# adr-arroyo/PointCloudComparator

Measured on AMD Instinct MI355X. Metric: nn_queries_per_sec, higher is better.
Workload: dtype f32; 1 GPU; C3: 10M x 10M XYZRGB (32-B stride), k=1 NN; step = index build over 10000000 references + 10000000 queries on each GPU (10000000 over 1 GPU); backend=none, engine=grid, references=10000000, queries_per_gpu=10000000, queries_total=10000000, point_stride_bytes=32

## Files before the change

pointcloudcomparator_amd/csrc/cellsort_mp.hip:

```cpp
#include "pcc_internal.hpp"
#include "grid_device.hpp"
#include "lane_ops.hpp"

namespace pcc {

constexpr int MP_T = 256;
constexpr unsigned int MP_F2 = 2048;
constexpr unsigned int MP_B2 = 128;
constexpr unsigned int MP_MAX_B1 = 256;
constexpr unsigned int MP_MAX_G = 512;
constexpr unsigned int MP_SLICE2 = 8192;
constexpr unsigned int MP_STAGE_BYTES = 32768;
constexpr unsigned int MP_WIN = 8;
#ifndef PCC_MP_STAGE_PTS
#define PCC_MP_STAGE_PTS 3072
#endif
#ifndef PCC_MP_STAGE_ORD
#define PCC_MP_STAGE_ORD 6144
#endif
constexpr unsigned int MP_FINE_STAGE_PTS = PCC_MP_STAGE_PTS, MP_FINE_STAGE_ORD = PCC_MP_STAGE_ORD;

struct MpPlan {
    unsigned int F1, F2, B1, G1, slice1;
};
static MpPlan mp_plan(unsigned int ncells_cap, unsigned int n) {
    MpPlan p;
    p.F2 = MP_F2;
    while ((unsigned long long)p.F2 * MP_B2 * MP_MAX_B1 < (unsigned long long)ncells_cap + 1) p.F2 *= 2;
    p.F1 = p.F2 * MP_B2;
    p.B1 = (ncells_cap + p.F1) / p.F1;
    p.G1 = (n + 16383) / 16384;
    if (p.G1 > MP_MAX_G) p.G1 = MP_MAX_G;
    if (p.G1 < 1) p.G1 = 1;
    p.slice1 = (n + p.G1 - 1) / p.G1;
    return p;
}

__device__ __forceinline__ unsigned int mp_cell(const float4& v, const GridParams& g, bool voxel) {
    return voxel ? voxel_id(v, g) : cell_id(v, g);
}
__device__ __forceinline__ unsigned int mp_cell(const uint2& v, const GridParams&, bool) { return v.x; }
__device__ __forceinline__ unsigned int mp_position(const float4& v) { return (unsigned int)__float_as_int(v.w); }
__device__ __forceinline__ unsigned int mp_position(const uint2& v) { return v.y; }
template <class E> __device__ __forceinline__ E mp_make(const float4& v, unsigned int cell);
template <> __device__ __forceinline__ float4 mp_make<float4>(const float4& v, unsigned int) { return v; }
template <> __device__ __forceinline__ uint2 mp_make<uint2>(const float4& v, unsigned int cell) {
    return make_uint2(cell, (unsigned int)__float_as_int(v.w));
}

__global__ void __launch_bounds__(MP_T)
k_mp_hist1(const float4* __restrict__ pts, unsigned int n, const GridDev* __restrict__ gd, unsigned int F1, unsigned int B1,
           unsigned int slice, unsigned int* __restrict__ H, unsigned int* __restrict__ zero, unsigned int n_zero) {
    for (unsigned int z = blockIdx.x * MP_T + threadIdx.x; z < n_zero; z += gridDim.x * MP_T) zero[z] = 0u;
    __shared__ unsigned int cnt[MP_MAX_B1];
    const GridParams g = gd->g;
    const bool voxel = gd->voxel != 0;
    for (unsigned int b = threadIdx.x; b < B1; b += MP_T) cnt[b] = 0;
    __syncthreads();
    const unsigned int beg = blockIdx.x * slice, end = min(n, beg + slice);
    for (unsigned int i0 = beg + threadIdx.x; i0 < end; i0 += 4 * MP_T) {
        float4 v[4];
#pragma unroll
        for (int u = 0; u < 4; ++u)
            if (i0 + u * MP_T < end) v[u] = pts[i0 + u * MP_T];
#pragma unroll
        for (int u = 0; u < 4; ++u)
            if (i0 + u * MP_T < end && __float_as_int(v[u].w) >= 0) atomicAdd(&cnt[mp_cell(v[u], g, voxel) / F1], 1u);
    }
    __syncthreads();
    for (unsigned int b = threadIdx.x; b < B1; b += MP_T) H[(size_t)b * gridDim.x + blockIdx.x] = cnt[b];
    if (blockIdx.x == 0 && threadIdx.x == 0) H[(size_t)B1 * gridDim.x] = 0;
}

template <class E>
__global__ void __launch_bounds__(MP_T)
k_mp_scatter1(const float4* __restrict__ pts, unsigned int n, const GridDev* __restrict__ gd, unsigned int F1, unsigned int B1,
              unsigned int slice, const unsigned int* __restrict__ H, E* __restrict__ out) {
    __shared__ unsigned int cur[MP_MAX_B1];
    const GridParams g = gd->g;
    const bool voxel = gd->voxel != 0;
    for (unsigned int b = threadIdx.x; b < B1; b += MP_T) cur[b] = H[(size_t)b * gridDim.x + blockIdx.x];
    __syncthreads();
    const unsigned int beg = blockIdx.x * slice, end = min(n, beg + slice);
    for (unsigned int i0 = beg + threadIdx.x; i0 < end; i0 += 4 * MP_T) {
        float4 v[4];
#pragma unroll
        for (int u = 0; u < 4; ++u)
            if (i0 + u * MP_T < end) v[u] = pts[i0 + u * MP_T];
#pragma unroll
        for (int u = 0; u < 4; ++u)
            if (i0 + u * MP_T < end && __float_as_int(v[u].w) >= 0) {
                const unsigned int c = mp_cell(v[u], g, voxel);
                out[atomicAdd(&cur[c / F1], 1u)] = mp_make<E>(v[u], c);
            }
    }
}

__global__ void __launch_bounds__(MP_T)
k_mp_hist1_cells(const unsigned int* __restrict__ cells, unsigned int n, unsigned int F1, unsigned int B1, unsigned int slice,
                 unsigned int* __restrict__ H, unsigned int* __restrict__ zero, unsigned int n_zero) {
    for (unsigned int z = blockIdx.x * MP_T + threadIdx.x; z < n_zero; z += gridDim.x * MP_T) zero[z] = 0u;
    __shared__ unsigned int cnt[MP_MAX_B1];
    for (unsigned int b = threadIdx.x; b < B1; b += MP_T) cnt[b] = 0;
    __syncthreads();
    const unsigned int beg = blockIdx.x * slice, end = min(n, beg + slice);
    for (unsigned int i0 = beg + threadIdx.x; i0 < end; i0 += 8 * MP_T) {
        unsigned int c[8];
#pragma unroll
        for (int u = 0; u < 8; ++u) c[u] = i0 + u * MP_T < end ? cells[i0 + u * MP_T] : 0xffffffffu;
#pragma unroll
        for (int u = 0; u < 8; ++u)
            if (c[u] != 0xffffffffu) atomicAdd(&cnt[c[u] / F1], 1u);
    }
    __syncthreads();
    for (unsigned int b = threadIdx.x; b < B1; b += MP_T) H[(size_t)b * gridDim.x + blockIdx.x] = cnt[b];
    if (blockIdx.x == 0 && threadIdx.x == 0) H[(size_t)B1 * gridDim.x] = 0;
}
__global__ void __launch_bounds__(MP_T)
k_mp_scatter1_cells(const unsigned int* __restrict__ cells, unsigned int n, unsigned int F1, unsigned int B1, unsigned int slice,
                    const unsigned int* __restrict__ H, uint2* __restrict__ out) {
    __shared__ unsigned int cur[MP_MAX_B1];
    for (unsigned int b = threadIdx.x; b < B1; b += MP_T) cur[b] = H[(size_t)b * gridDim.x + blockIdx.x];
    __syncthreads();
    const unsigned int beg = blockIdx.x * slice, end = min(n, beg + slice);
    for (unsigned int i0 = beg + threadIdx.x; i0 < end; i0 += 8 * MP_T) {
        unsigned int c[8];
#pragma unroll
        for (int u = 0; u < 8; ++u) c[u] = i0 + u * MP_T < end ? cells[i0 + u * MP_T] : 0xffffffffu;
#pragma unroll
        for (int u = 0; u < 8; ++u)
            if (c[u] != 0xffffffffu) out[atomicAdd(&cur[c[u] / F1], 1u)] = make_uint2(c[u], i0 + u * MP_T);
    }
}

constexpr unsigned int MP_TILE1 = 2048;
template <class E>
__global__ void __launch_bounds__(MP_T)
k_mp_scatter1_staged(const float4* __restrict__ pts, unsigned int n, const GridDev* __restrict__ gd, unsigned int F1, unsigned int B1,
                     unsigned int slice, const unsigned int* __restrict__ H, E* __restrict__ out) {
    constexpr int PER = MP_TILE1 / MP_T;
    __shared__ unsigned int cur[MP_MAX_B1], tcnt[MP_MAX_B1], tstart[MP_MAX_B1];
    __shared__ unsigned short sb[MP_TILE1];
    __shared__ __attribute__((aligned(16))) unsigned char stage_raw[MP_TILE1 * sizeof(E)];
    E* stage = reinterpret_cast<E*>(stage_raw);
    const GridParams g = gd->g;
    const bool voxel = gd->voxel != 0;
    for (unsigned int b = threadIdx.x; b < B1; b += MP_T) cur[b] = H[(size_t)b * gridDim.x + blockIdx.x];
    const unsigned int beg = blockIdx.x * slice, end = min(n, beg + slice);
    for (unsigned int t0 = beg; t0 < end; t0 += MP_TILE1) {
        for (unsigned int b = threadIdx.x; b < MP_MAX_B1; b += MP_T) tcnt[b] = 0;
        __syncthreads();
        float4 v[PER];
        unsigned int bk[PER], rk[PER];
#pragma unroll
        for (int u = 0; u < PER; ++u) {
            const unsigned int i = t0 + threadIdx.x + u * MP_T;
            v[u] = make_float4(0.f, 0.f, 0.f, __int_as_float(-1));
            if (i < end) v[u] = pts[i];
        }
#pragma unroll
        for (int u = 0; u < PER; ++u) {
            bk[u] = 0xffffffffu;
            rk[u] = 0;
            if (__float_as_int(v[u].w) >= 0) {
                bk[u] = mp_cell(v[u], g, voxel);
                rk[u] = atomicAdd(&tcnt[bk[u] / F1], 1u);
            }
        }
        __syncthreads();
        if (threadIdx.x < 64) {
            unsigned int c[4], sum = 0;
#pragma unroll
            for (int j = 0; j < 4; ++j) { c[j] = tcnt[4 * threadIdx.x + j]; sum += c[j]; }
            unsigned int ex = wave_incl_scan_add(sum) - sum;
#pragma unroll
            for (int j = 0; j < 4; ++j) { tstart[4 * threadIdx.x + j] = ex; ex += c[j]; }
        }
        __syncthreads();
#pragma unroll
        for (int u = 0; u < PER; ++u)
            if (bk[u] != 0xffffffffu) {
                const unsigned int b = bk[u] / F1, slot = tstart[b] + rk[u];
                stage[slot] = mp_make<E>(v[u], bk[u]);
                sb[slot] = (unsigned short)b;
            }
        __syncthreads();
        const unsigned int tile_n = tstart[MP_MAX_B1 - 1] + tcnt[MP_MAX_B1 - 1];
        for (unsigned int j = threadIdx.x; j < tile_n; j += MP_T) {
            const unsigned int b = sb[j];
            out[cur[b] + (j - tstart[b])] = stage[j];
        }
        __syncthreads();
        for (unsigned int b = threadIdx.x; b < MP_MAX_B1; b += MP_T) cur[b] += tcnt[b];
    }
}

__device__ __forceinline__ unsigned int mp_pair(unsigned int c, unsigned int F1, unsigned int F2) {
    return (c / F1) * MP_B2 + (c % F1) / F2;
}

template <bool PLACE, class E>
__global__ void __launch_bounds__(MP_T)
k_mp_level2(const E* __restrict__ in, const unsigned int* __restrict__ n_valid_ptr, const GridDev* __restrict__ gd,
            unsigned int F1, unsigned int F2, unsigned int* __restrict__ C, E* __restrict__ out) {
    constexpr unsigned int SLICE = PLACE ? MP_STAGE_BYTES / sizeof(E) : MP_SLICE2;
    __shared__ unsigned int cnt[MP_WIN * MP_B2];
    __shared__ __attribute__((aligned(16))) unsigned char stage_raw[PLACE ? MP_STAGE_BYTES : 16];
    E* stage = reinterpret_cast<E*>(stage_raw);
    const GridParams g = gd->g;
    const bool voxel = gd->voxel != 0;
    const unsigned int n = *n_valid_ptr;
    const unsigned int beg = blockIdx.x * SLICE, end = min(n, beg + SLICE);
    if (beg >= end) return;
    const unsigned int w0 = (mp_cell(in[beg], g, voxel) / F1) * MP_B2;
    for (unsigned int k = threadIdx.x; k < MP_WIN * MP_B2; k += MP_T) cnt[k] = 0;
    __syncthreads();
    for (unsigned int i0 = beg + threadIdx.x; i0 < end; i0 += 4 * MP_T) {
        E v[4];
#pragma unroll
        for (int u = 0; u < 4; ++u)
            if (i0 + u * MP_T < end) v[u] = in[i0 + u * MP_T];
#pragma unroll
        for (int u = 0; u < 4; ++u) {
            if (i0 + u * MP_T >= end) break;
            if (PLACE) stage[i0 + u * MP_T - beg] = v[u];
            const unsigned int pr = mp_pair(mp_cell(v[u], g, voxel), F1, F2);
            if (pr - w0 < MP_WIN * MP_B2) atomicAdd(&cnt[pr - w0], 1u);
            else if (!PLACE) atomicAdd(&C[pr], 1u);
            else out[atomicAdd(&C[pr], 1u)] = v[u];
        }
    }
    __syncthreads();
    for (unsigned int k = threadIdx.x; k < MP_WIN * MP_B2; k += MP_T) {
        const unsigned int c = cnt[k];
        if (c) {
            if (!PLACE) atomicAdd(&C[w0 + k], c);
            else cnt[k] = atomicAdd(&C[w0 + k], c);
        }
    }
    if (!PLACE) return;
    __syncthreads();
    for (unsigned int j = threadIdx.x; j < end - beg; j += MP_T) {
        const E v = stage[j];
        const unsigned int pr = mp_pair(mp_cell(v, g, voxel), F1, F2);
        if (pr - w0 < MP_WIN * MP_B2) out[atomicAdd(&cnt[pr - w0], 1u)] = v;
    }
}

__device__ __forceinline__ void mp_store_point(float4* out, unsigned int pos, const float4& v) { if (out) out[pos] = v; }
__device__ __forceinline__ void mp_store_point(float4*, unsigned int, const uint2&) {}

template <bool REFS, class E>
__global__ void __launch_bounds__(MP_T)
k_mp_fine(const E* __restrict__ in, const unsigned int* __restrict__ ends , const GridDev* __restrict__ gd,
          unsigned int F2, float4* __restrict__ out_pts, unsigned int* __restrict__ out_order,
          unsigned int* __restrict__ cell_start) {
    extern __shared__ __attribute__((aligned(16))) unsigned int lds[];
    unsigned int* cnt = lds;
    unsigned int* wsum = lds + F2;
    const GridParams g = gd->g;
    const bool voxel = gd->voxel != 0;
    const unsigned int ncells = (unsigned int)g.ncells;
    const unsigned int b = blockIdx.x;
    const unsigned int cell0 = b * F2;
    if (cell0 > ncells) return;
    const unsigned int beg = b ? ends[b - 1] : 0u, end = ends[b];
    if (!REFS && beg == end) return;
    for (unsigned int f = threadIdx.x; f < F2; f += MP_T) cnt[f] = 0;
    __syncthreads();
    for (unsigned int j0 = beg + threadIdx.x; j0 < end; j0 += 4 * MP_T) {
        E v[4];
#pragma unroll
        for (int u = 0; u < 4; ++u)
            if (j0 + u * MP_T < end) v[u] = in[j0 + u * MP_T];
#pragma unroll
        for (int u = 0; u < 4; ++u)
            if (j0 + u * MP_T < end) atomicAdd(&cnt[mp_cell(v[u], g, voxel) - cell0], 1u);
    }
    __syncthreads();
    const unsigned int per = (F2 + MP_T - 1) / MP_T;
    const unsigned int f0 = threadIdx.x * per, f1 = min(F2, f0 + per);
    unsigned int s = 0;
    for (unsigned int f = f0; f < f1; ++f) s += cnt[f];
    const unsigned int lane = threadIdx.x & 63, wave = threadIdx.x >> 6;
    const unsigned int inc = wave_incl_scan_add(s);
    if (lane == 63) wsum[wave] = inc;
    __syncthreads();
    unsigned int run = beg + inc - s;
    for (unsigned int w = 0; w < wave; ++w) run += wsum[w];
    for (unsigned int f = f0; f < f1; ++f) {
        const unsigned int c = cnt[f];
        cnt[f] = run;
        if (REFS && cell0 + f <= ncells) cell_start[cell0 + f] = run;
        run += c;
    }
    __syncthreads();
    const unsigned int stage_cap = out_pts ? MP_FINE_STAGE_PTS : MP_FINE_STAGE_ORD;
    const bool staged = end - beg <= stage_cap;
    float4* st_pts = reinterpret_cast<float4*>(lds + ((F2 + 4 + 3) & ~3u));
    unsigned int* st_ord = reinterpret_cast<unsigned int*>(st_pts + (out_pts ? MP_FINE_STAGE_PTS : 0));
    for (unsigned int j0 = beg + threadIdx.x; j0 < end; j0 += 4 * MP_T) {
        E v[4];
#pragma unroll
        for (int u = 0; u < 4; ++u)
            if (j0 + u * MP_T < end) v[u] = in[j0 + u * MP_T];
#pragma unroll
        for (int u = 0; u < 4; ++u) {
            if (j0 + u * MP_T >= end) break;
            const unsigned int pos = atomicAdd(&cnt[mp_cell(v[u], g, voxel) - cell0], 1u);
            if (staged) {
                mp_store_point(out_pts ? st_pts : nullptr, pos - beg, v[u]);
                if (out_order) st_ord[pos - beg] = mp_position(v[u]);
            } else {
                mp_store_point(out_pts, pos, v[u]);
                if (out_order) out_order[pos] = mp_position(v[u]);
            }
        }
    }
    if (staged) {
        __syncthreads();
        for (unsigned int i = threadIdx.x; i < end - beg; i += MP_T) {
            if (out_pts) out_pts[beg + i] = st_pts[i];
            if (out_order) out_order[beg + i] = st_ord[i];
        }
    }
}

int cell_sort_mp(pcc_index* ix, const float4* pts, size_t n_pts, bool refs, float4* out_pts, unsigned int* out_order,
                 unsigned int* cell_start, unsigned int** n_sorted_dev, const GridDev* gd_override,
                 unsigned int nc_cap_override) {
    hipStream_t s = ix->stream;
    const unsigned int n = (unsigned int)n_pts;
    const unsigned int ncap = gd_override ? nc_cap_override : ix->nc_cap;
    const MpPlan p = mp_plan(ncap, n);
    const GridDev* gd = gd_override ? gd_override : ix->d_grid.as<GridDev>();
    const unsigned int np = p.B1 * MP_B2;
    PCC_TRY(ix->mp_a.reserve((size_t)n * sizeof(float4) + 256));
    PCC_TRY(ix->mp_b.reserve((size_t)n * sizeof(float4) + 256));
    const size_t h_elems = (size_t)p.B1 * p.G1 + 1;
    PCC_TRY(ix->scratch_b.reserve(((h_elems + 3) & ~(size_t)3) * sizeof(unsigned int)));
    PCC_TRY(ix->mp_c.reserve(((size_t)np + 8) * sizeof(unsigned int)));
    unsigned int* H = ix->scratch_b.as<unsigned int>();
    unsigned int* C = ix->mp_c.as<unsigned int>();
    const unsigned int* cells = nullptr;
    if (!refs && !out_pts && !gd_override && pts == ix->q_packed.as<float4>() && ix->q_cells_n == n_pts && n_pts != 0)
        cells = ix->q_cells.as<unsigned int>();
    if (!refs) ix->q_cells_n = 0;
    if (cells)
        hipLaunchKernelGGL(k_mp_hist1_cells, dim3(p.G1), dim3(MP_T), 0, s, cells, n, p.F1, p.B1, p.slice1, H, C, np);
    else
    hipLaunchKernelGGL(k_mp_hist1, dim3(p.G1), dim3(MP_T), 0, s, pts, n, gd, p.F1, p.B1, p.slice1, H, C, np);
    PCC_HIP(hipGetLastError());
    PCC_TRY(launch_exclusive_scan(ix, s, H, h_elems, ix->scratch_a));
    unsigned int* n_valid = H + h_elems - 1;
    if (n_sorted_dev) *n_sorted_dev = n_valid;
    const size_t lds3 = (((size_t)p.F2 + 4 + 3) & ~(size_t)3) * sizeof(unsigned int) +
                        (out_pts ? (size_t)MP_FINE_STAGE_PTS * (sizeof(float4) + (out_order ? sizeof(unsigned int) : 0))
                                 : (size_t)MP_FINE_STAGE_ORD * sizeof(unsigned int));
    const unsigned int g2c = (n + MP_SLICE2 - 1) / MP_SLICE2;
    if (out_pts) {
        float4* t1 = ix->mp_a.as<float4>();
        float4* t2 = ix->mp_b.as<float4>();
        const unsigned int g2p = (n + MP_STAGE_BYTES / sizeof(float4) - 1) / (MP_STAGE_BYTES / sizeof(float4));
        if (ix->opt.sort_stage1)
            hipLaunchKernelGGL((k_mp_scatter1_staged<float4>), dim3(p.G1), dim3(MP_T), 0, s, pts, n, gd, p.F1, p.B1, p.slice1, H, t1);
        else
            hipLaunchKernelGGL((k_mp_scatter1<float4>), dim3(p.G1), dim3(MP_T), 0, s, pts, n, gd, p.F1, p.B1, p.slice1, H, t1);
        hipLaunchKernelGGL((k_mp_level2<false, float4>), dim3(g2c), dim3(MP_T), 0, s, t1, n_valid, gd, p.F1, p.F2, C, t2);
        PCC_TRY(launch_exclusive_scan(ix, s, C, np, ix->scratch_a));
        hipLaunchKernelGGL((k_mp_level2<true, float4>), dim3(g2p), dim3(MP_T), 0, s, t1, n_valid, gd, p.F1, p.F2, C, t2);
        if (refs)
            hipLaunchKernelGGL((k_mp_fine<true, float4>), dim3(np), dim3(MP_T), lds3, s, t2, C, gd, p.F2, out_pts, out_order, cell_start);
        else
            hipLaunchKernelGGL((k_mp_fine<false, float4>), dim3(np), dim3(MP_T), lds3, s, t2, C, gd, p.F2, out_pts, out_order, cell_start);
    } else {
        uint2* t1 = ix->mp_a.as<uint2>();
        uint2* t2 = ix->mp_b.as<uint2>();
        const unsigned int g2p = (n + MP_STAGE_BYTES / sizeof(uint2) - 1) / (MP_STAGE_BYTES / sizeof(uint2));
        if (cells)
            hipLaunchKernelGGL(k_mp_scatter1_cells, dim3(p.G1), dim3(MP_T), 0, s, cells, n, p.F1, p.B1, p.slice1, H, t1);
        else if (ix->opt.sort_stage1 == 2)
            hipLaunchKernelGGL((k_mp_scatter1_staged<uint2>), dim3(p.G1), dim3(MP_T), 0, s, pts, n, gd, p.F1, p.B1, p.slice1, H, t1);
        else
            hipLaunchKernelGGL((k_mp_scatter1<uint2>), dim3(p.G1), dim3(MP_T), 0, s, pts, n, gd, p.F1, p.B1, p.slice1, H, t1);
        hipLaunchKernelGGL((k_mp_level2<false, uint2>), dim3(g2c), dim3(MP_T), 0, s, t1, n_valid, gd, p.F1, p.F2, C, t2);
        PCC_TRY(launch_exclusive_scan(ix, s, C, np, ix->scratch_a));
        hipLaunchKernelGGL((k_mp_level2<true, uint2>), dim3(g2p), dim3(MP_T), 0, s, t1, n_valid, gd, p.F1, p.F2, C, t2);
        if (refs)
            hipLaunchKernelGGL((k_mp_fine<true, uint2>), dim3(np), dim3(MP_T), lds3, s, t2, C, gd, p.F2, out_pts, out_order, cell_start);
        else
            hipLaunchKernelGGL((k_mp_fine<false, uint2>), dim3(np), dim3(MP_T), lds3, s, t2, C, gd, p.F2, out_pts, out_order, cell_start);
    }
    PCC_HIP(hipGetLastError());
    return PCC_OK;
}

}
```

Before: 7.377 billion queries/s.

## Rewrite level-2 placement as locally-sorted staged scatter with 1024-thread blocks

```diff
diff --git a/pointcloudcomparator_amd/csrc/cellsort_mp.hip b/pointcloudcomparator_amd/csrc/cellsort_mp.hip
--- a/pointcloudcomparator_amd/csrc/cellsort_mp.hip
+++ b/pointcloudcomparator_amd/csrc/cellsort_mp.hip
@@ -10,8 +10,10 @@
 constexpr unsigned int MP_MAX_B1 = 256;
 constexpr unsigned int MP_MAX_G = 512;
 constexpr unsigned int MP_SLICE2 = 8192;
-constexpr unsigned int MP_STAGE_BYTES = 32768;
 constexpr unsigned int MP_WIN = 8;
+constexpr unsigned int MP_T2 = 1024;
+constexpr unsigned int MP_PLACE_PTS = 2048;
+constexpr unsigned int MP_PLACE_PAIRS = 4096;
 #ifndef PCC_MP_STAGE_PTS
 #define PCC_MP_STAGE_PTS 3072
 #endif
@@ -199,13 +201,51 @@
     return (c / F1) * MP_B2 + (c % F1) / F2;
 }
 
-template <bool PLACE, class E>
-__global__ void __launch_bounds__(MP_T)
-k_mp_level2(const E* __restrict__ in, const unsigned int* __restrict__ n_valid_ptr, const GridDev* __restrict__ gd,
+template <class E>
+__global__ void __launch_bounds__(MP_T)
+k_mp_count2(const E* __restrict__ in, const unsigned int* __restrict__ n_valid_ptr, const GridDev* __restrict__ gd,
+            unsigned int F1, unsigned int F2, unsigned int* __restrict__ C) {
+    __shared__ unsigned int cnt[MP_WIN * MP_B2];
+    const GridParams g = gd->g;
+    const bool voxel = gd->voxel != 0;
+    const unsigned int n = *n_valid_ptr;
+    const unsigned int beg = blockIdx.x * MP_SLICE2, end = min(n, beg + MP_SLICE2);
+    if (beg >= end) return;
+    const unsigned int w0 = (mp_cell(in[beg], g, voxel) / F1) * MP_B2;
+    for (unsigned int k = threadIdx.x; k < MP_WIN * MP_B2; k += MP_T) cnt[k] = 0;
+    __syncthreads();
+    for (unsigned int i0 = beg + threadIdx.x; i0 < end; i0 += 4 * MP_T) {
+        E v[4];
+#pragma unroll
+        for (int u = 0; u < 4; ++u)
+            if (i0 + u * MP_T < end) v[u] = in[i0 + u * MP_T];
+#pragma unroll
+        for (int u = 0; u < 4; ++u) {
+            if (i0 + u * MP_T >= end) break;
+            const unsigned int pr = mp_pair(mp_cell(v[u], g, voxel), F1, F2);
+            if (pr - w0 < MP_WIN * MP_B2) atomicAdd(&cnt[pr - w0], 1u);
+            else atomicAdd(&C[pr], 1u);
+        }
+    }
+    __syncthreads();
+    for (unsigned int k = threadIdx.x; k < MP_WIN * MP_B2; k += MP_T) {
+        const unsigned int c = cnt[k];
+        if (c) atomicAdd(&C[w0 + k], c);
+    }
+}
+
+template <class E, unsigned int SLICE>
+__global__ void __launch_bounds__(MP_T2)
+k_mp_place2(const E* __restrict__ in, const unsigned int* __restrict__ n_valid_ptr, const GridDev* __restrict__ gd,
             unsigned int F1, unsigned int F2, unsigned int* __restrict__ C, E* __restrict__ out) {
-    constexpr unsigned int SLICE = PLACE ? MP_STAGE_BYTES / sizeof(E) : MP_SLICE2;
-    __shared__ unsigned int cnt[MP_WIN * MP_B2];
-    __shared__ __attribute__((aligned(16))) unsigned char stage_raw[PLACE ? MP_STAGE_BYTES : 16];
+    constexpr int PER = SLICE / MP_T2;
+    constexpr unsigned int NW = MP_WIN * MP_B2;
+    static_assert(SLICE % MP_T2 == 0 && SLICE <= 65536 && NW == MP_T2, "bucket and rank share a word; one window counter per thread");
+    __shared__ unsigned int cnt[NW];
+    __shared__ unsigned int delta[NW];
+    __shared__ unsigned int wsum[MP_T2 / 64 + 1];
+    __shared__ unsigned short sb[SLICE];
+    __shared__ __attribute__((aligned(16))) unsigned char stage_raw[SLICE * sizeof(E)];
     E* stage = reinterpret_cast<E*>(stage_raw);
     const GridParams g = gd->g;
     const bool voxel = gd->voxel != 0;
@@ -213,38 +253,47 @@
     const unsigned int beg = blockIdx.x * SLICE, end = min(n, beg + SLICE);
     if (beg >= end) return;
     const unsigned int w0 = (mp_cell(in[beg], g, voxel) / F1) * MP_B2;
-    for (unsigned int k = threadIdx.x; k < MP_WIN * MP_B2; k += MP_T) cnt[k] = 0;
-    __syncthreads();
-    for (unsigned int i0 = beg + threadIdx.x; i0 < end; i0 += 4 * MP_T) {
-        E v[4];
-#pragma unroll
-        for (int u = 0; u < 4; ++u)
-            if (i0 + u * MP_T < end) v[u] = in[i0 + u * MP_T];
-#pragma unroll
-        for (int u = 0; u < 4; ++u) {
-            if (i0 + u * MP_T >= end) break;
-            if (PLACE) stage[i0 + u * MP_T - beg] = v[u];
-            const unsigned int pr = mp_pair(mp_cell(v[u], g, voxel), F1, F2);
-            if (pr - w0 < MP_WIN * MP_B2) atomicAdd(&cnt[pr - w0], 1u);
-            else if (!PLACE) atomicAdd(&C[pr], 1u);
-            else out[atomicAdd(&C[pr], 1u)] = v[u];
-        }
-    }
-    __syncthreads();
-    for (unsigned int k = threadIdx.x; k < MP_WIN * MP_B2; k += MP_T) {
-        const unsigned int c = cnt[k];
-        if (c) {
-            if (!PLACE) atomicAdd(&C[w0 + k], c);
-            else cnt[k] = atomicAdd(&C[w0 + k], c);
-        }
-    }
-    if (!PLACE) return;
-    __syncthreads();
-    for (unsigned int j = threadIdx.x; j < end - beg; j += MP_T) {
-        const E v = stage[j];
-        const unsigned int pr = mp_pair(mp_cell(v, g, voxel), F1, F2);
-        if (pr - w0 < MP_WIN * MP_B2) out[atomicAdd(&cnt[pr - w0], 1u)] = v;
-    }
+    cnt[threadIdx.x] = 0;
+    __syncthreads();
+    E v[PER];
+    unsigned int br[PER];
+#pragma unroll
+    for (int u = 0; u < PER; ++u) {
+        const unsigned int i = beg + threadIdx.x + u * MP_T2;
+        if (i < end) v[u] = in[i];
+    }
+#pragma unroll
+    for (int u = 0; u < PER; ++u) {
+        br[u] = 0xffffffffu;
+        if (beg + threadIdx.x + u * MP_T2 < end) {
+            const unsigned int k = mp_pair(mp_cell(v[u], g, voxel), F1, F2) - w0;
+            if (k < NW) br[u] = (k << 16) | atomicAdd(&cnt[k], 1u);
+            else out[atomicAdd(&C[w0 + k], 1u)] = v[u];
+        }
+    }
+    __syncthreads();
+    const unsigned int c = cnt[threadIdx.x];
+    const unsigned int gbase = c ? atomicAdd(&C[w0 + threadIdx.x], c) : 0u;
+    const unsigned int lane = threadIdx.x & 63, wave = threadIdx.x >> 6;
+    const unsigned int inc = wave_incl_scan_add(c);
+    if (lane == 63) wsum[wave] = inc;
+    __syncthreads();
+    unsigned int lstart = inc - c;
+    for (unsigned int w = 0; w < wave; ++w) lstart += wsum[w];
+    cnt[threadIdx.x] = lstart;
+    delta[threadIdx.x] = gbase - lstart;
+    if (threadIdx.x == MP_T2 - 1) wsum[MP_T2 / 64] = lstart + c;
+    __syncthreads();
+#pragma unroll
+    for (int u = 0; u < PER; ++u)
+        if (br[u] != 0xffffffffu) {
+            const unsigned int k = br[u] >> 16, slot = cnt[k] + (br[u] & 0xffffu);
+            stage[slot] = v[u];
+            sb[slot] = (unsigned short)k;
+        }
+    __syncthreads();
+    const unsigned int staged = wsum[MP_T2 / 64];
+    for (unsigned int j = threadIdx.x; j < staged; j += MP_T2) out[delta[sb[j]] + j] = stage[j];
 }
 
 __device__ __forceinline__ void mp_store_point(float4* out, unsigned int pos, const float4& v) { if (out) out[pos] = v; }
@@ -361,14 +410,14 @@
     if (out_pts) {
         float4* t1 = ix->mp_a.as<float4>();
         float4* t2 = ix->mp_b.as<float4>();
-        const unsigned int g2p = (n + MP_STAGE_BYTES / sizeof(float4) - 1) / (MP_STAGE_BYTES / sizeof(float4));
+        const unsigned int g2p = (n + MP_PLACE_PTS - 1) / MP_PLACE_PTS;
         if (ix->opt.sort_stage1)
             hipLaunchKernelGGL((k_mp_scatter1_staged<float4>), dim3(p.G1), dim3(MP_T), 0, s, pts, n, gd, p.F1, p.B1, p.slice1, H, t1);
         else
             hipLaunchKernelGGL((k_mp_scatter1<float4>), dim3(p.G1), dim3(MP_T), 0, s, pts, n, gd, p.F1, p.B1, p.slice1, H, t1);
-        hipLaunchKernelGGL((k_mp_level2<false, float4>), dim3(g2c), dim3(MP_T), 0, s, t1, n_valid, gd, p.F1, p.F2, C, t2);
+        hipLaunchKernelGGL((k_mp_count2<float4>), dim3(g2c), dim3(MP_T), 0, s, t1, n_valid, gd, p.F1, p.F2, C);
         PCC_TRY(launch_exclusive_scan(ix, s, C, np, ix->scratch_a));
-        hipLaunchKernelGGL((k_mp_level2<true, float4>), dim3(g2p), dim3(MP_T), 0, s, t1, n_valid, gd, p.F1, p.F2, C, t2);
+        hipLaunchKernelGGL((k_mp_place2<float4, MP_PLACE_PTS>), dim3(g2p), dim3(MP_T2), 0, s, t1, n_valid, gd, p.F1, p.F2, C, t2);
         if (refs)
             hipLaunchKernelGGL((k_mp_fine<true, float4>), dim3(np), dim3(MP_T), lds3, s, t2, C, gd, p.F2, out_pts, out_order, cell_start);
         else
@@ -376,16 +425,16 @@
     } else {
         uint2* t1 = ix->mp_a.as<uint2>();
         uint2* t2 = ix->mp_b.as<uint2>();
-        const unsigned int g2p = (n + MP_STAGE_BYTES / sizeof(uint2) - 1) / (MP_STAGE_BYTES / sizeof(uint2));
+        const unsigned int g2p = (n + MP_PLACE_PAIRS - 1) / MP_PLACE_PAIRS;
         if (cells)
             hipLaunchKernelGGL(k_mp_scatter1_cells, dim3(p.G1), dim3(MP_T), 0, s, cells, n, p.F1, p.B1, p.slice1, H, t1);
         else if (ix->opt.sort_stage1 == 2)
             hipLaunchKernelGGL((k_mp_scatter1_staged<uint2>), dim3(p.G1), dim3(MP_T), 0, s, pts, n, gd, p.F1, p.B1, p.slice1, H, t1);
         else
             hipLaunchKernelGGL((k_mp_scatter1<uint2>), dim3(p.G1), dim3(MP_T), 0, s, pts, n, gd, p.F1, p.B1, p.slice1, H, t1);
-        hipLaunchKernelGGL((k_mp_level2<false, uint2>), dim3(g2c), dim3(MP_T), 0, s, t1, n_valid, gd, p.F1, p.F2, C, t2);
+        hipLaunchKernelGGL((k_mp_count2<uint2>), dim3(g2c), dim3(MP_T), 0, s, t1, n_valid, gd, p.F1, p.F2, C);
         PCC_TRY(launch_exclusive_scan(ix, s, C, np, ix->scratch_a));
-        hipLaunchKernelGGL((k_mp_level2<true, uint2>), dim3(g2p), dim3(MP_T), 0, s, t1, n_valid, gd, p.F1, p.F2, C, t2);
+        hipLaunchKernelGGL((k_mp_place2<uint2, MP_PLACE_PAIRS>), dim3(g2p), dim3(MP_T2), 0, s, t1, n_valid, gd, p.F1, p.F2, C, t2);
         if (refs)
             hipLaunchKernelGGL((k_mp_fine<true, uint2>), dim3(np), dim3(MP_T), lds3, s, t2, C, gd, p.F2, out_pts, out_order, cell_start);
         else
```

Result: faster. 7.581 billion queries/s, median of 6 (+2.8%).
